# rrahn/libspm

Hardware: AMD Instinct MI355X
Metric: Gbases/s scanned, Myers k<=3 |P|=100 (higher is better)
Workload: dtype u32

## Files before the change

### libspm_amd/csrc/filter_verify.hip

```cpp
#include "filter_launch.hpp"
#include "filter_verify.hpp"

namespace
{
template <int NWN>
void launch_verify_nw(const verify_params &V, dim3 grid, hipStream_t s)
{
    uint32_t threads = 256;
    const size_t per_thread = (size_t)(V.sigma + 1) * NWN * 4 + 2 * 16;
    while (threads > 64 && per_thread * threads > 128 * 1024)
        threads >>= 1;
    const size_t lds = per_thread * threads + (size_t)(threads / 64) * kHitStage * sizeof(spm_hit);
    launch(verify_kernel<NWN>, grid, threads, lds, s, V);
}

template <int G>
void launch_verify_wave_g(verify_params V, const uint32_t *peq_bot, uint32_t max_m, dim3 grid, hipStream_t s)
{
    grid.x *= 4;
    const uint32_t n_slots = 2 * V.max_k + 1 + V.max_span;
    V.wave_text = ((max_m + V.max_k + n_slots + 16 + 15) & ~15u) + 16;
    const size_t per_group = ((n_slots * 2 + 15) & ~15u) + V.wave_text;
    launch(verify_wave_kernel<G, 1>, grid, 64, (64 / G) * per_group, s, V, peq_bot);
}
}

void launch_band_runs(const verify_params &V, band_rec *bands, band_rec *heads, unsigned long long *head_count, uint32_t n_cu,
                      hipStream_t s)
{
    hipLaunchKernelGGL(band_runs_kernel, dim3(n_cu * 8), dim3(256), 0, s, V, bands, heads, head_count);
}

void launch_band_select(const verify_params &V, band_rec *out, unsigned long long *out_count, uint32_t n_cu, hipStream_t s)
{
    hipLaunchKernelGGL(band_select_kernel, dim3(n_cu * 2), dim3(256), 0, s, V, out, out_count);
}

void launch_band_release(const verify_params &V, const band_rec *bands, uint32_t n_cu, hipStream_t s)
{
    hipLaunchKernelGGL(band_release_kernel, dim3(n_cu * 8), dim3(256), 0, s, V, bands, (uint32_t)kCntBandSlots);
}

void launch_verify_wave(uint32_t n_blocks, const verify_params &V, const uint32_t *peq_bot, uint32_t max_m, uint32_t n_cu,
                        hipStream_t s)
{
    const dim3 grid(n_cu * 16);
    if (n_blocks <= 8)
        launch_verify_wave_g<8>(V, peq_bot, max_m, grid, s);
    else if (n_blocks <= 16)
        launch_verify_wave_g<16>(V, peq_bot, max_m, grid, s);
    else if (n_blocks <= 32)
        launch_verify_wave_g<32>(V, peq_bot, max_m, grid, s);
    else
        launch_verify_wave_g<64>(V, peq_bot, max_m, grid, s);
}

void launch_verify(uint32_t nwn, const verify_params &V, uint64_t band_expect, uint32_t n_cu, hipStream_t s)
{
    const dim3 grid((uint32_t)std::min<uint64_t>((uint64_t)n_cu * 4, std::max<uint64_t>(n_cu / 2, (band_expect + 255) / 256)));
    switch (nwn) {
    case 1: launch_verify_nw<1>(V, grid, s); break;
    case 2: launch_verify_nw<2>(V, grid, s); break;
    case 3: launch_verify_nw<3>(V, grid, s); break;
    case 4: launch_verify_nw<4>(V, grid, s); break;
    case 5: launch_verify_nw<5>(V, grid, s); break;
    case 6: launch_verify_nw<6>(V, grid, s); break;
    case 7: launch_verify_nw<7>(V, grid, s); break;
    case 8: launch_verify_nw<8>(V, grid, s); break;
    case 16: launch_verify_nw<16>(V, grid, s); break;
    case 32: launch_verify_nw<32>(V, grid, s); break;
    default: launch_verify_nw<64>(V, grid, s); break;
    }
}

void warm_verify_kernels()
{
    hipFuncAttributes a;
    (void)hipFuncGetAttributes(&a, (const void *)band_release_kernel);
}
```

### libspm_amd/csrc/filter_verify.hpp

```cpp
#pragma once

#include "brute.hpp"
#include "filter_params.hpp"
#include "pack.hpp"
#include "wave.hpp"

namespace spm_hip
{

__device__ __forceinline__ bool seen_insert(const verify_params &P, uint32_t pat, int64_t e)
{
    return seen_insert_raw(P.seen, P.seen_mask, P.overflow, pat, e);
}

__global__ __launch_bounds__(256) void band_select_kernel(const verify_params P, band_rec *out, unsigned long long *out_count)
{
    unsigned long long n = P.counters[kCntBandSlots];
    if (n > P.band_cap)
        n = P.band_cap;
    const uint32_t lane = threadIdx.x & 63;
    const uint64_t stride = (uint64_t)gridDim.x * blockDim.x;
    const uint64_t rounds = (n + stride - 1) / stride;
    for (uint64_t r = 0; r < rounds; ++r) {
        const uint64_t i = r * stride + (uint64_t)blockIdx.x * blockDim.x + threadIdx.x;
        bool keep = false;
        band_rec c;
        c.val = kBandInvalid;
        if (i < n) {
            c = P.bands[i];
            if (c.val != kBandInvalid) {
                const uint32_t cnt = (uint32_t)band_value(P.band_tab[c.slot].y, true);
                band_release(P.band_tab, c.slot);
                keep = cnt >= (P.surplus ? (uint32_t)P.surplus[c.val >> 11] : 1u);
            }
        }
        const uint64_t m = __ballot(keep);
        if (m != 0) {
            unsigned long long base = 0;
            const int leader = __ffsll((unsigned long long)m) - 1;
            if ((int)lane == leader)
                base = atomicAdd(out_count, (unsigned long long)__popcll(m));
            base = __shfl(base, leader);
            if (keep)
                out[base + __popcll(m & ((1ull << lane) - 1))] = c;
        }
    }
}

constexpr uint32_t kRunAnalysed = 0x400u;
constexpr uint32_t kRunFollower = 0x200u;
constexpr uint32_t kRunLenShift = 5, kRunLenMask = 0x3u, kRunHiMask = 0x1Fu;
constexpr uint32_t kRunTouchLeft = 0x80u, kRunTouchRight = 0x100u;
constexpr uint32_t kRunMax = 4;

__device__ __forceinline__ uint32_t band_lookup(const verify_params &P, unsigned long long bkey)
{
    uint32_t s2 = (uint32_t)mix64(bkey) & P.table_mask;
    for (uint32_t tries = 0; tries < 8192; ++tries) {
        const unsigned long long o = P.band_tab[s2].x;
        if (o == bkey)
            return s2;
        if (o == kBandEmpty)
            return 0xFFFFFFFFu;
        s2 = (s2 + 1) & P.table_mask;
    }
    return 0xFFFFFFFFu;
}

__global__ __launch_bounds__(256) void band_runs_kernel(const verify_params P, band_rec *bands, band_rec *heads,
                                                        unsigned long long *head_count)
{
    __shared__ uint32_t wave_tot01[4], wave_tot23[4];
    __shared__ unsigned long long chunk_base;
    unsigned long long n = P.counters[P.band_counter];
    if (n > P.band_cap)
        n = P.band_cap;
    constexpr uint32_t PER = 8;
    const uint32_t tid = threadIdx.x, lane = tid & 63, wave = tid >> 6;
    for (uint64_t c0 = (uint64_t)blockIdx.x * (256 * PER); c0 < n; c0 += (uint64_t)gridDim.x * (256 * PER)) {
        band_rec mine[PER];
        uint32_t head_mask = 0, cnt = 0;
#pragma unroll
        for (uint32_t j = 0; j < PER; ++j) {
            const uint64_t i = c0 + (uint64_t)j * 256 + tid;
            mine[j].val = kBandInvalid;
            if (i >= n)
                continue;
            band_rec c = bands[i];
            if (c.val == kBandInvalid)
                continue;
            const unsigned long long base = ((unsigned long long)(c.val >> 11) << 43) | ((unsigned long long)c.seg << P.band_bits);
            uint32_t code = kRunAnalysed;
            const bool pred = c.band > 0 && band_lookup(P, base | (unsigned long long)(c.band - 1)) != 0xFFFFFFFFu;
            if (c.band % kRunMax != 0 && pred) {
                code |= kRunFollower;
            } else {
                uint32_t followers = 0, last = c.slot;
                bool cut = true;
                for (uint32_t r = 1; r < kRunMax && (c.band + r) % kRunMax != 0; ++r) {
                    const uint32_t s2 = band_lookup(P, base | (unsigned long long)(c.band + r));
                    if (s2 == 0xFFFFFFFFu) {
                        cut = false;
                        break;
                    }
                    followers = r;
                    last = s2;
                }
                const bool succ = cut && band_lookup(P, base | (unsigned long long)(c.band + followers + 1)) != 0xFFFFFFFFu;
                const unsigned long long v = band_value(P.band_tab[last].y, false);
                const uint32_t hi = v ? (uint32_t)(63 - __clzll((long long)v)) : 0u;
                code |= (followers << kRunLenShift) | (hi & kRunHiMask) | (pred ? kRunTouchLeft : 0u) | (succ ? kRunTouchRight : 0u);
                head_mask |= 1u << j;
                ++cnt;
            }
            c.val = (c.val & ~0x7FFu) | code;
            mine[j] = c;
        }
        uint32_t c01 = 0, c23 = 0;
#pragma unroll
        for (uint32_t j = 0; j < PER; ++j)
            if (head_mask & (1u << j)) {
                const uint32_t cls = (mine[j].val >> kRunLenShift) & kRunLenMask;
                const uint32_t one = 1u << (16 * (cls & 1u));
                c01 += cls < 2 ? one : 0u;
                c23 += cls < 2 ? 0u : one;
            }
        uint32_t i01 = c01, i23 = c23;
#pragma unroll
        for (int o = 1; o < 64; o <<= 1) {
            const uint32_t u01 = (uint32_t)__shfl_up((int)i01, o), u23 = (uint32_t)__shfl_up((int)i23, o);
            if (lane >= (uint32_t)o) {
                i01 += u01;
                i23 += u23;
            }
        }
        if (lane == 63) {
            wave_tot01[wave] = i01;
            wave_tot23[wave] = i23;
        }
        __syncthreads();
        uint32_t off01 = 0, off23 = 0, tot01 = 0, tot23 = 0;
        for (uint32_t w = 0; w < 4; ++w) {
            off01 += w < wave ? wave_tot01[w] : 0u;
            off23 += w < wave ? wave_tot23[w] : 0u;
            tot01 += wave_tot01[w];
            tot23 += wave_tot23[w];
        }
        const uint32_t tot[4] = {tot01 & 0xFFFFu, tot01 >> 16, tot23 & 0xFFFFu, tot23 >> 16};
        const uint32_t total = tot[0] + tot[1] + tot[2] + tot[3];
        if (tid == 0)
            chunk_base = total ? atomicAdd(head_count, (unsigned long long)total) : 0ull;
        __syncthreads();
        const uint32_t mine_before[4] = {(off01 & 0xFFFFu) + ((i01 - c01) & 0xFFFFu), (off01 >> 16) + ((i01 - c01) >> 16),
                                         (off23 & 0xFFFFu) + ((i23 - c23) & 0xFFFFu), (off23 >> 16) + ((i23 - c23) >> 16)};
        uint64_t pos[4];
        pos[0] = chunk_base + mine_before[0];
        pos[1] = chunk_base + tot[0] + mine_before[1];
        pos[2] = chunk_base + tot[0] + tot[1] + mine_before[2];
        pos[3] = chunk_base + tot[0] + tot[1] + tot[2] + mine_before[3];
#pragma unroll
        for (uint32_t j = 0; j < PER; ++j)
            if (head_mask & (1u << j)) {
                const uint32_t cls = (mine[j].val >> kRunLenShift) & kRunLenMask;
                const uint64_t at = cls == 0 ? pos[0] : cls == 1 ? pos[1] : cls == 2 ? pos[2] : pos[3];
                heads[at] = mine[j];
                pos[0] += cls == 0 ? 1u : 0u;
                pos[1] += cls == 1 ? 1u : 0u;
                pos[2] += cls == 2 ? 1u : 0u;
                pos[3] += cls == 3 ? 1u : 0u;
            }
        __syncthreads();
    }
}

__global__ __launch_bounds__(256) void band_release_kernel(const verify_params P, const band_rec *bands, uint32_t counter)
{
    unsigned long long n = P.counters[counter];
    if (n > P.band_cap)
        n = P.band_cap;
    const uint64_t stride = (uint64_t)gridDim.x * blockDim.x;
    for (uint64_t i = (uint64_t)blockIdx.x * blockDim.x + threadIdx.x; i < n; i += stride) {
        const band_rec c = bands[i];
        if (c.val != kBandInvalid)
            band_release(P.band_tab, c.slot);
    }
}

struct band_geom
{
    uint32_t pat;
    int64_t m, k;
    int64_t e_lo, e_hi;
    int64_t ws;
    int64_t dd_lo, dd_hi;
};

__device__ __forceinline__ bool decode_band(const verify_params &P, const band_rec &c, bool consume, band_geom &g)
{
    if (c.val == kBandInvalid)
        return false;
    g.pat = c.val >> 11;
    unsigned long long v = 1;
    if (!P.preselected) {
        v = band_value(P.band_tab[c.slot].y, P.overlap != 0);
        if (consume)
            band_release(P.band_tab, c.slot);
        if (c.val & kRunFollower)
            return false;
        if (P.overlap ? (uint32_t)v < (P.surplus ? (uint32_t)P.surplus[g.pat] : 1u) : v == 0)
            return false;
    }
    g.m = P.m[g.pat];
    g.k = P.k[g.pat];
    int64_t own_b = (int64_t)P.scan_begin, own_e = (int64_t)P.scan_end, hay_b = (int64_t)P.ctx_begin;
    if (P.seg_offsets) {
        const int64_t sb = (int64_t)P.seg_offsets[c.seg], se = (int64_t)P.seg_offsets[c.seg + 1];
        own_b = P.seg_owned ? sb + (int64_t)P.seg_owned[c.seg] : sb;
        own_e = se;
        hay_b = sb;
    }
    const int64_t band_base = hay_b - (int64_t)P.max_m + (int64_t)c.band * (int64_t)P.Bw;
    int64_t d = band_base;
    int64_t span = (int64_t)P.Bw - 1 + (P.overlap ? g.k + 1 : 0);
    if (!P.overlap) {
        const int lo = __ffsll((long long)v) - 1;
        int hi = 63 - __clzll((long long)v);
        if (c.val & kRunAnalysed)
            hi = (int)(((c.val >> kRunLenShift) & kRunLenMask) * P.Bw + (c.val & kRunHiMask));
        d += lo;
        span = hi - lo;
    }
    g.e_lo = d + g.m - g.k;
    g.e_hi = d + g.m + g.k + span;
    g.dd_lo = INT64_MAX;
    g.dd_hi = INT64_MIN;
    if (!P.overlap && (c.val & kRunAnalysed) && !P.seg_offsets) {
        const int64_t next_base = band_base + (int64_t)(((c.val >> kRunLenShift) & kRunLenMask) + 1) * (int64_t)P.Bw;
        g.dd_lo = (c.val & kRunTouchLeft) ? band_base + g.m + g.k : INT64_MIN;
        g.dd_hi = (c.val & kRunTouchRight) ? next_base + g.m - g.k - 1 : INT64_MAX;
    }
    if (g.e_lo < own_b + 1)
        g.e_lo = own_b + 1;
    if (g.e_hi > own_e)
        g.e_hi = own_e;
    if (g.e_lo > g.e_hi)
        return false;
    g.ws = g.e_lo - (g.m + g.k);
    if (g.ws < hay_b)
        g.ws = hay_b;
    return true;
}

template <int NWN>
__global__ __launch_bounds__(256) void verify_kernel(const verify_params P)
{
    extern __shared__ uint32_t vlds[];
    const uint32_t tid = threadIdx.x;
    const uint32_t nthr = blockDim.x;
    const uint32_t rows = P.sigma + 1;
    uint16_t *hitbuf = reinterpret_cast<uint16_t *>(vlds + (size_t)rows * NWN * nthr);
    spm_hit *stage = reinterpret_cast<spm_hit *>(hitbuf + (size_t)16 * nthr) + (size_t)(tid >> 6) * kHitStage;
    uint32_t n_staged = 0;
    const uint32_t lane = tid & 63;
    auto flush = [&]() {
        if (n_staged == 0)
            return;
        unsigned long long base = 0;
        if (lane == 0)
            base = atomicAdd(P.hit_counter, (unsigned long long)n_staged);
        base = uniform_u64(base);
        for (uint32_t i = lane; i < n_staged; i += 64)
            if (base + i < P.hit_cap)
                P.hits[base + i] = stage[i];
        n_staged = 0;
        queue_sync();
    };
    unsigned long long n_cand = P.counters[P.band_counter];
    if (n_cand > P.band_cap)
        n_cand = P.band_cap;
    const uint64_t stride = (uint64_t)gridDim.x * nthr;
    uint32_t n_valid = 0;
    const uint64_t rounds = (n_cand + stride - 1) / stride;
    for (uint64_t rd = 0; rd < rounds; ++rd) {
        const uint64_t ci = rd * stride + (uint64_t)blockIdx.x * nthr + tid;
        band_geom g;
        g.pat = 0;
        g.m = 1;
        g.k = 0;
        g.e_lo = 0;
        g.e_hi = -1;
        g.ws = 0;
        const bool active = ci < n_cand && decode_band(P, P.bands[ci], P.runs == 0, g);
        if (active)
            ++n_valid;
        const uint32_t pat = g.pat;
        const int64_t m = g.m, k = g.k, e_lo = g.e_lo, e_hi = active ? g.e_hi : g.ws, ws = g.ws;
        const uint32_t *src = P.peq32 + (((size_t)(pat >> 6) * rows) * P.nw_table + (P.nw_table - NWN)) * 64 + (pat & 63);
        if (active)
            for (uint32_t r = 0; r < rows; ++r)
#pragma unroll
                for (int w = 0; w < NWN; ++w)
                    vlds[((size_t)r * NWN + w) * nthr + tid] = src[((size_t)r * P.nw_table + w) * 64];
        myers_lane<NWN, false> L;
        {
            const int32_t off = NWN * 32 - (int32_t)m;
#pragma unroll
            for (int w = 0; w < NWN; ++w) {
                const int32_t lo = off - w * 32;
                L.VP[w] = lo <= 0 ? 0xFFFFFFFFu : (lo >= 32 ? 0u : (0xFFFFFFFFu << lo));
                L.VN[w] = 0;
            }
            L.score = (int32_t)m;
        }
        const int64_t blk0 = ws & ~15ll;
        uint4 nxt = make_uint4(0, 0, 0, 0);
        if (active)
            nxt = load_text16(P.text, (uint64_t)blk0, P.text_alloc);
        const uint32_t n_cols = (uint32_t)(e_hi - ws);
        const uint32_t rel_lo = (uint32_t)(e_lo - 1 - ws);
        const uint32_t sigma = P.sigma;
        uint32_t rel0 = (uint32_t)(blk0 - ws);
        const uint32_t my_blocks = active ? (uint32_t)((e_hi - blk0 + 15) >> 4) : 0u;
        uint32_t max_blocks = my_blocks;
        for (int o = 32; o > 0; o >>= 1)
            max_blocks = max(max_blocks, (uint32_t)__shfl_xor((int)max_blocks, o));
        max_blocks = (uint32_t)__builtin_amdgcn_readfirstlane(max_blocks);
        for (uint32_t bi = 0; bi < max_blocks; ++bi, rel0 += 16) {
            const int64_t blk = blk0 + 16 * (int64_t)bi;
            uint32_t hitmask = 0;
            if (bi < my_blocks) {
                const uint4 cur = nxt;
                if (bi + 1 < my_blocks)
                    nxt = load_text16(P.text, (uint64_t)(blk + 16), P.text_alloc);
                const uint32_t words[4] = {cur.x, cur.y, cur.z, cur.w};
#pragma unroll
                for (int i = 0; i < 16; ++i) {
                    const uint32_t rel = rel0 + (uint32_t)i;
                    if (rel >= n_cols)
                        continue;
                    uint32_t sym = (words[i >> 2] >> (8 * (i & 3))) & 0xFF;
                    sym = sym < sigma ? sym : sigma;
                    L.step_strided(vlds + ((size_t)sym * NWN) * nthr + tid, nthr);
                    if (L.score <= (int32_t)k && rel >= rel_lo) {
                        hitbuf[(size_t)i * nthr + tid] = (uint16_t)(L.score + 1);
                        hitmask |= 1u << i;
                    }
                }
            }
            if (__ballot(hitmask != 0) == 0)
                continue;
            uint32_t fresh = 0, keep = 0;
            for (uint32_t mm = hitmask; mm != 0; mm &= mm - 1) {
                const uint32_t i = (uint32_t)__ffs(mm) - 1u;
                const int64_t e = blk + (int64_t)i + 1;
                if ((e > g.dd_lo && e < g.dd_hi) || seen_insert(P, pat, e)) {
                    ++fresh;
                    keep |= 1u << i;
                }
            }
            uint32_t incl = fresh;
#pragma unroll
            for (int o = 1; o < 64; o <<= 1) {
                const uint32_t up = (uint32_t)__shfl_up((int)incl, o);
                if (lane >= (uint32_t)o)
                    incl += up;
            }
            const uint32_t total = (uint32_t)__builtin_amdgcn_readfirstlane(__shfl((int)incl, 63));
            if (total == 0)
                continue;
            if (n_staged + total > kHitStage)
                flush();
            unsigned long long direct = 0;
            const bool staged = total <= kHitStage;
            if (!staged) {
                if (lane == 0)
                    direct = atomicAdd(P.hit_counter, (unsigned long long)total);
                direct = uniform_u64(direct);
            }
            uint32_t at = n_staged + incl - fresh;
            for (uint32_t mm = keep; mm != 0; mm &= mm - 1) {
                const uint32_t i = (uint32_t)__ffs(mm) - 1u;
                const int64_t e = blk + (int64_t)i + 1;
                spm_hit h;
                h.pos = (P.report_begin ? (uint64_t)(e - m) : (uint64_t)e) + P.pos_offset;
                h.pattern = pat;
                h.score = (int32_t)hitbuf[(size_t)i * nthr + tid] - 1;
                if (staged)
                    stage[at] = h;
                else if (direct + at < P.hit_cap)
                    P.hits[direct + at] = h;
                ++at;
            }
            if (staged)
                n_staged += total;
            queue_sync();
        }
    }
    flush();
    wave_count_add(P.hit_counter + kCntBandsVerified, n_valid);
}


template <int G, int NB>
__global__ __launch_bounds__(256) void verify_wave_kernel(const verify_params P, const uint32_t *__restrict__ peq_bot)
{
    extern __shared__ uint16_t whit[];
    constexpr uint32_t GPW = 64 / G;
    const uint32_t lane = threadIdx.x & 63, gl = lane & (G - 1), gw = lane / G;
    const uint32_t wave = threadIdx.x >> 6, waves = blockDim.x >> 6;
    const uint32_t n_slots = 2 * P.max_k + 1 + P.max_span;
    const uint32_t group_bytes = ((n_slots * 2 + 15) & ~15u) + P.wave_text;
    uint8_t *gbase = reinterpret_cast<uint8_t *>(whit) + (size_t)(wave * GPW + gw) * group_bytes;
    uint16_t *hb = reinterpret_cast<uint16_t *>(gbase);
    uint8_t *tw = gbase + ((n_slots * 2 + 15) & ~15u);
    for (uint32_t r = gl; r < n_slots; r += G)
        hb[r] = 0;
    unsigned long long n_cand = P.counters[P.band_counter];
    if (n_cand > P.band_cap)
        n_cand = P.band_cap;
    const uint64_t stride = (uint64_t)gridDim.x * waves * GPW;
    const uint32_t rows = P.sigma + 1;
    uint32_t n_valid = 0;
    for (uint64_t base = ((uint64_t)blockIdx.x * waves + wave) * GPW; base < n_cand; base += stride) {
        const uint64_t ci = base + gw;
        bool active = ci < n_cand;
        uint32_t pat = 0;
        int64_t m = 1, k = 0, e_lo = 0, e_hi = -1, ws = 0;
        band_rec c;
        c.val = kBandInvalid;
        c.slot = 0;
        if (active)
            c = P.bands[ci];
        {
            band_geom g;
            g.pat = 0;
            g.m = 1;
            g.k = 0;
            g.e_lo = 0;
            g.e_hi = -1;
            g.ws = 0;
            active = active && decode_band(P, c, false, g);
            pat = g.pat;
            m = g.m;
            k = g.k;
            e_lo = g.e_lo;
            e_hi = g.e_hi;
            ws = g.ws;
        }
        __builtin_amdgcn_wave_barrier();
        if (gl == 0 && c.val != kBandInvalid && !P.preselected)
            band_release(P.band_tab, c.slot);
        if (active && gl == 0)
            ++n_valid;
        const uint32_t nbk = (uint32_t)((m + 31) >> 5);
        const uint32_t nb = (nbk + NB - 1) / NB;
        const uint32_t n_cols = active ? (uint32_t)(e_hi - ws) : 0u;
        const bool mine = active && gl < nb;
        const bool lane_last = gl + 1 == nb;
        const uint32_t j_last = (nbk - 1) % NB;
        uint32_t out_bit[NB];
#pragma unroll
        for (int j = 0; j < NB; ++j)
            out_bit[j] = (gl * NB + (uint32_t)j + 1 == nbk) ? (uint32_t)((m - 1) & 31) : 31u;
        const uint32_t skew = (uint32_t)(ws & 15);
        uint32_t beyond4 = 0;
        if (active) {
            const uint32_t n_bytes = (skew + n_cols + 15) & ~15u;
            for (uint32_t off = gl * 16; off < n_bytes; off += G * 16) {
                const uint4 v = load_text16(P.text, ((uint64_t)ws & ~15ull) + off, P.text_alloc);
                *reinterpret_cast<uint4 *>(tw + off) = v;
                beyond4 |= (v.x | v.y | v.z | v.w) & 0xFCFCFCFCu;
            }
        }
        const bool plain4 = P.sigma == 4 && __ballot(beyond4 != 0) == 0;
        uint32_t e0[NB], e1[NB], e2[NB], e3[NB], e4[NB];
#pragma unroll
        for (int j = 0; j < NB; ++j) {
            e0[j] = e1[j] = e2[j] = e3[j] = e4[j] = 0;
            const uint32_t gb = gl * NB + (uint32_t)j;
            if (mine && gb < nbk) {
                const uint32_t *src = peq_bot + (((size_t)(pat >> 6) * rows) * P.nw_table + gb) * 64 + (pat & 63);
                const size_t rs = (size_t)P.nw_table * 64;
                e0[j] = src[0];
                e1[j] = src[rs];
                e2[j] = P.sigma > 2 ? src[2 * rs] : 0u;
                e3[j] = P.sigma > 3 ? src[3 * rs] : 0u;
                e4[j] = P.sigma > 4 ? src[4 * rs] : 0u;
            }
        }
        queue_sync();
        uint32_t Pv[NB], Mv[NB], ho = 0;
#pragma unroll
        for (int j = 0; j < NB; ++j) {
            Pv[j] = 0xFFFFFFFFu;
            Mv[j] = 0;
        }
        int32_t score = (int32_t)m;
        bool any_hit = false;
        const uint32_t first_slot_col = (uint32_t)(e_lo - ws) - 1;
        const uint32_t t_end = n_cols + nb - 1;
        uint32_t t_wave = active ? t_end : 0u;
        uint32_t t_lo = active ? nb - 1 : 0u, t_hi = active ? n_cols : 0xFFFFFFFFu;
        uint32_t t_hit = active ? first_slot_col + nb - 1 : 0xFFFFFFFFu;
        for (int o = 32; o >= (int)G; o >>= 1) {
            t_wave = max(t_wave, (uint32_t)__shfl_xor((int)t_wave, o));
            t_lo = max(t_lo, (uint32_t)__shfl_xor((int)t_lo, o));
            t_hi = min(t_hi, (uint32_t)__shfl_xor((int)t_hi, o));
            t_hit = min(t_hit, (uint32_t)__shfl_xor((int)t_hit, o));
        }
        t_wave = (uint32_t)__builtin_amdgcn_readfirstlane(t_wave);
        t_lo = (uint32_t)__builtin_amdgcn_readfirstlane(t_lo);
        t_hi = (uint32_t)__builtin_amdgcn_readfirstlane(t_hi);
        t_hit = (uint32_t)__builtin_amdgcn_readfirstlane(t_hit);
        t_hi = t_hi > t_wave ? t_wave : t_hi;
        t_lo = t_lo > t_hi ? t_hi : t_lo;
        t_hit = t_hit < t_lo ? t_lo : (t_hit > t_hi ? t_hi : t_hit);
        uint32_t sym_next = mine ? tw[skew] : 0u;
        const uint8_t *my_text = mine ? tw + skew - gl : tw;
        const int32_t k_hit = (lane_last && mine) ? (int32_t)k : -1;
        const uint32_t n_rel = n_cols - first_slot_col;
        auto step = [&](uint32_t t, auto checked, auto dna4, auto hits) {
            const uint32_t ho_up = (uint32_t)__builtin_amdgcn_update_dpp(0, (int)ho, 0x138, 0xF, 0xF, false);
            const uint32_t col = t - gl;
            const uint32_t sym = sym_next;
            if constexpr (decltype(checked)::value) {
                uint32_t nc = col + 1;
                nc = nc < n_cols ? nc : 0u;
                sym_next = tw[skew + nc];
            } else {
                sym_next = my_text[t + 1];
            }
            if (!decltype(checked)::value || (mine && col < n_cols)) {
                uint32_t hin = gl == 0 ? 0u : ho_up;
                uint32_t s0 = 0, s1 = 0;
                if constexpr (decltype(dna4)::value) {
                    s0 = (uint32_t)((int32_t)(sym << 31) >> 31);
                    s1 = (uint32_t)((int32_t)(sym << 30) >> 31);
                }
                int32_t d_last = 0;
#pragma unroll
                for (int j = 0; j < NB; ++j) {
                    uint32_t Eq;
                    if constexpr (decltype(dna4)::value) {
                        const uint32_t lo2 = (e1[j] & s0) | (e0[j] & ~s0), hi2 = (e3[j] & s0) | (e2[j] & ~s0);
                        Eq = (hi2 & s1) | (lo2 & ~s1);
                    } else {
                        const uint32_t lo2 = (sym & 1u) ? e1[j] : e0[j], hi2 = (sym & 1u) ? e3[j] : e2[j];
                        Eq = (sym & 2u) ? hi2 : lo2;
                        Eq = sym < 4 ? Eq : (sym == 4 ? e4[j] : 0u);
                        Eq = sym < P.sigma ? Eq : 0u;
                    }
                    const uint32_t hp = hin & 1u, hn = hin >> 1;
                    const uint32_t Xv = Eq | Mv[j];
                    Eq |= hn;
                    const uint32_t Xh = (((Eq & Pv[j]) + Pv[j]) ^ Pv[j]) | Eq;
                    uint32_t Ph = Mv[j] | ~(Xh | Pv[j]);
                    uint32_t Mh = Pv[j] & Xh;
                    const uint32_t op = (Ph >> out_bit[j]) & 1u, on = (Mh >> out_bit[j]) & 1u;
                    hin = op | (on << 1);
                    Ph = (Ph << 1) | hp;
                    Mh = (Mh << 1) | hn;
                    Pv[j] = Mh | ~(Xv | Ph);
                    Mv[j] = Ph & Xv;
                    if (NB == 1 || (uint32_t)j == j_last)
                        d_last = (int32_t)op - (int32_t)on;
                }
                ho = hin;
                score += d_last;
                if constexpr (decltype(hits)::value) {
                    const uint32_t rel = col - first_slot_col;
                    if (score <= k_hit && rel < n_rel) {
                        hb[rel] = (uint16_t)(score + 1);
                        any_hit = true;
                    }
                }
            }
        };
        uint32_t t = 0;
        for (; t < t_lo; ++t)
            step(t, std::true_type{}, std::false_type{}, std::true_type{});
        if (plain4) {
            for (; t < t_hit; ++t)
                step(t, std::false_type{}, std::true_type{}, std::false_type{});
            for (; t < t_hi; ++t)
                step(t, std::false_type{}, std::true_type{}, std::true_type{});
        } else {
            for (; t < t_hi; ++t)
                step(t, std::false_type{}, std::false_type{}, std::true_type{});
        }
        for (; t < t_wave; ++t)
            step(t, std::true_type{}, std::false_type{}, std::true_type{});
        queue_sync();
        if (__ballot(any_hit) != 0) {
            const uint32_t nr = active ? (uint32_t)(e_hi - e_lo) + 1 : 0u;
            uint32_t fresh = 0;
            for (uint32_t r = gl; r < nr; r += G) {
                const uint32_t sc1 = hb[r];
                if (sc1) {
                    if (seen_insert(P, pat, e_lo + (int64_t)r))
                        ++fresh;
                    else
                        hb[r] = 0;
                }
            }
            unsigned long long idx = wave_reserve_hits(P.hit_counter, fresh);
            for (uint32_t r = gl; r < nr; r += G) {
                const uint32_t sc1 = hb[r];
                hb[r] = 0;
                if (sc1) {
                    if (idx < P.hit_cap) {
                        const int64_t e = e_lo + (int64_t)r;
                        spm_hit h;
                        h.pos = (P.report_begin ? (uint64_t)(e - m) : (uint64_t)e) + P.pos_offset;
                        h.pattern = pat;
                        h.score = (int32_t)sc1 - 1;
                        P.hits[idx] = h;
                    }
                    ++idx;
                }
            }
        }
        queue_sync();
    }
    wave_count_add(P.hit_counter + kCntBandsVerified, n_valid);
}

}
```

Before: 6533.

## Replace register Eq select with LDS symbol table lookup in wave verify kernel

The wave verify kernel now stores each lane's per-symbol pattern-match words in an LDS table indexed by symbol, replacing the register-held e0..e4 arrays and the branchless select logic. Text bytes are clamped so out-of-range symbols map to a zero row, which removes the separate DNA4/plain path. The Eq word for the next column is prefetched one step ahead, the horizontal carries pass as separate DPP values with sign-extended bit extraction, and the unchecked loop is manually unrolled by four. The NB multi-block-per-lane template is dropped. This adds LDS traffic per step and extra table storage per launch, in exchange for fewer ALU ops in the inner recurrence.

```diff
diff --git a/libspm_amd/csrc/filter_verify.hip b/libspm_amd/csrc/filter_verify.hip
--- a/libspm_amd/csrc/filter_verify.hip
+++ b/libspm_amd/csrc/filter_verify.hip
@@ -21,7 +21,7 @@
     const uint32_t n_slots = 2 * V.max_k + 1 + V.max_span;
     V.wave_text = ((max_m + V.max_k + n_slots + 16 + 15) & ~15u) + 16;
     const size_t per_group = ((n_slots * 2 + 15) & ~15u) + V.wave_text;
-    launch(verify_wave_kernel<G, 1>, grid, 64, (64 / G) * per_group, s, V, peq_bot);
+    launch(verify_wave_kernel<G>, grid, 64, (64 / G) * per_group + kWaveTableBytes, s, V, peq_bot);
 }
 }
 
diff --git a/libspm_amd/csrc/filter_verify.hpp b/libspm_amd/csrc/filter_verify.hpp
--- a/libspm_amd/csrc/filter_verify.hpp
+++ b/libspm_amd/csrc/filter_verify.hpp
@@ -401,7 +401,18 @@
 }
 
 
-template <int G, int NB>
+constexpr uint32_t kWaveSymRows = 8;
+constexpr uint32_t kWaveTableBytes = kWaveSymRows * 64 * 4;
+
+__device__ __forceinline__ uint32_t clamp_syms(uint32_t w)
+{
+    const uint32_t hi = w & 0xF8F8F8F8u;
+    const uint32_t any = ((hi | (hi >> 1) | (hi >> 2) | (hi >> 3) | (hi >> 4)) >> 3) & 0x01010101u;
+    const uint32_t full = any * 0xFFu;
+    return (w & ~full) | (0x07070707u & full);
+}
+
+template <int G>
 __global__ __launch_bounds__(256) void verify_wave_kernel(const verify_params P, const uint32_t *__restrict__ peq_bot)
 {
     extern __shared__ uint16_t whit[];
@@ -413,8 +424,12 @@
     uint8_t *gbase = reinterpret_cast<uint8_t *>(whit) + (size_t)(wave * GPW + gw) * group_bytes;
     uint16_t *hb = reinterpret_cast<uint16_t *>(gbase);
     uint8_t *tw = gbase + ((n_slots * 2 + 15) & ~15u);
+    uint32_t *tabl = reinterpret_cast<uint32_t *>(reinterpret_cast<uint8_t *>(whit) + (size_t)waves * GPW * group_bytes +
+                                                  (size_t)wave * kWaveTableBytes) + lane;
     for (uint32_t r = gl; r < n_slots; r += G)
         hb[r] = 0;
+    for (uint32_t off = gl * 16; off < P.wave_text; off += G * 16)
+        *reinterpret_cast<uint4 *>(tw + off) = make_uint4(0, 0, 0, 0);
     unsigned long long n_cand = P.counters[P.band_counter];
     if (n_cand > P.band_cap)
         n_cand = P.band_cap;
@@ -452,49 +467,31 @@
             band_release(P.band_tab, c.slot);
         if (active && gl == 0)
             ++n_valid;
-        const uint32_t nbk = (uint32_t)((m + 31) >> 5);
-        const uint32_t nb = (nbk + NB - 1) / NB;
+        const uint32_t nb = (uint32_t)((m + 31) >> 5);
         const uint32_t n_cols = active ? (uint32_t)(e_hi - ws) : 0u;
         const bool mine = active && gl < nb;
         const bool lane_last = gl + 1 == nb;
-        const uint32_t j_last = (nbk - 1) % NB;
-        uint32_t out_bit[NB];
-#pragma unroll
-        for (int j = 0; j < NB; ++j)
-            out_bit[j] = (gl * NB + (uint32_t)j + 1 == nbk) ? (uint32_t)((m - 1) & 31) : 31u;
+        const uint32_t out_bit = lane_last ? (uint32_t)((m - 1) & 31) : 31u;
         const uint32_t skew = (uint32_t)(ws & 15);
-        uint32_t beyond4 = 0;
         if (active) {
             const uint32_t n_bytes = (skew + n_cols + 15) & ~15u;
             for (uint32_t off = gl * 16; off < n_bytes; off += G * 16) {
-                const uint4 v = load_text16(P.text, ((uint64_t)ws & ~15ull) + off, P.text_alloc);
+                uint4 v = load_text16(P.text, ((uint64_t)ws & ~15ull) + off, P.text_alloc);
+                if ((v.x | v.y | v.z | v.w) & 0xF8F8F8F8u)
+                    v = make_uint4(clamp_syms(v.x), clamp_syms(v.y), clamp_syms(v.z), clamp_syms(v.w));
                 *reinterpret_cast<uint4 *>(tw + off) = v;
-                beyond4 |= (v.x | v.y | v.z | v.w) & 0xFCFCFCFCu;
-            }
-        }
-        const bool plain4 = P.sigma == 4 && __ballot(beyond4 != 0) == 0;
-        uint32_t e0[NB], e1[NB], e2[NB], e3[NB], e4[NB];
-#pragma unroll
-        for (int j = 0; j < NB; ++j) {
-            e0[j] = e1[j] = e2[j] = e3[j] = e4[j] = 0;
-            const uint32_t gb = gl * NB + (uint32_t)j;
-            if (mine && gb < nbk) {
-                const uint32_t *src = peq_bot + (((size_t)(pat >> 6) * rows) * P.nw_table + gb) * 64 + (pat & 63);
-                const size_t rs = (size_t)P.nw_table * 64;
-                e0[j] = src[0];
-                e1[j] = src[rs];
-                e2[j] = P.sigma > 2 ? src[2 * rs] : 0u;
-                e3[j] = P.sigma > 3 ? src[3 * rs] : 0u;
-                e4[j] = P.sigma > 4 ? src[4 * rs] : 0u;
-            }
+            }
+        }
+        {
+            const uint32_t *src = peq_bot + (((size_t)(pat >> 6) * rows) * P.nw_table + gl) * 64 + (pat & 63);
+            const size_t rs = (size_t)P.nw_table * 64;
+#pragma unroll
+            for (uint32_t r = 0; r < kWaveSymRows; ++r)
+                tabl[r * 64] = (mine && r < P.sigma) ? src[r * rs] : 0u;
         }
         queue_sync();
-        uint32_t Pv[NB], Mv[NB], ho = 0;
-#pragma unroll
-        for (int j = 0; j < NB; ++j) {
-            Pv[j] = 0xFFFFFFFFu;
-            Mv[j] = 0;
-        }
+        uint32_t Pv = 0xFFFFFFFFu, Mv = 0;
+        uint32_t op_c = 0, on_c = 0;
         int32_t score = (int32_t)m;
         bool any_hit = false;
         const uint32_t first_slot_col = (uint32_t)(e_lo - ws) - 1;
@@ -515,58 +512,38 @@
         t_hi = t_hi > t_wave ? t_wave : t_hi;
         t_lo = t_lo > t_hi ? t_hi : t_lo;
         t_hit = t_hit < t_lo ? t_lo : (t_hit > t_hi ? t_hi : t_hit);
-        uint32_t sym_next = mine ? tw[skew] : 0u;
         const uint8_t *my_text = mine ? tw + skew - gl : tw;
         const int32_t k_hit = (lane_last && mine) ? (int32_t)k : -1;
         const uint32_t n_rel = n_cols - first_slot_col;
-        auto step = [&](uint32_t t, auto checked, auto dna4, auto hits) {
-            const uint32_t ho_up = (uint32_t)__builtin_amdgcn_update_dpp(0, (int)ho, 0x138, 0xF, 0xF, false);
+        const uint32_t carry_in = gl == 0 ? 0u : 1u;
+        uint32_t eq_cur = tabl[(uint32_t)tw[skew] * 64];
+        uint32_t sym_nx = tw[skew + ((1u - gl) < n_cols ? 1u - gl : 0u)];
+        auto step = [&](uint32_t t, auto checked, auto hits) {
             const uint32_t col = t - gl;
-            const uint32_t sym = sym_next;
+            const uint32_t eq_nx = tabl[sym_nx * 64];
             if constexpr (decltype(checked)::value) {
-                uint32_t nc = col + 1;
+                uint32_t nc = col + 2;
                 nc = nc < n_cols ? nc : 0u;
-                sym_next = tw[skew + nc];
+                sym_nx = tw[skew + nc];
             } else {
-                sym_next = my_text[t + 1];
-            }
+                sym_nx = my_text[t + 2];
+            }
+            const uint32_t hp = (uint32_t)__builtin_amdgcn_update_dpp(0, (int)op_c, 0x138, 0xF, 0xF, true) & carry_in;
+            const uint32_t hn = (uint32_t)__builtin_amdgcn_update_dpp(0, (int)on_c, 0x138, 0xF, 0xF, true) & carry_in;
             if (!decltype(checked)::value || (mine && col < n_cols)) {
-                uint32_t hin = gl == 0 ? 0u : ho_up;
-                uint32_t s0 = 0, s1 = 0;
-                if constexpr (decltype(dna4)::value) {
-                    s0 = (uint32_t)((int32_t)(sym << 31) >> 31);
-                    s1 = (uint32_t)((int32_t)(sym << 30) >> 31);
-                }
-                int32_t d_last = 0;
-#pragma unroll
-                for (int j = 0; j < NB; ++j) {
-                    uint32_t Eq;
-                    if constexpr (decltype(dna4)::value) {
-                        const uint32_t lo2 = (e1[j] & s0) | (e0[j] & ~s0), hi2 = (e3[j] & s0) | (e2[j] & ~s0);
-                        Eq = (hi2 & s1) | (lo2 & ~s1);
-                    } else {
-                        const uint32_t lo2 = (sym & 1u) ? e1[j] : e0[j], hi2 = (sym & 1u) ? e3[j] : e2[j];
-                        Eq = (sym & 2u) ? hi2 : lo2;
-                        Eq = sym < 4 ? Eq : (sym == 4 ? e4[j] : 0u);
-                        Eq = sym < P.sigma ? Eq : 0u;
-                    }
-                    const uint32_t hp = hin & 1u, hn = hin >> 1;
-                    const uint32_t Xv = Eq | Mv[j];
-                    Eq |= hn;
-                    const uint32_t Xh = (((Eq & Pv[j]) + Pv[j]) ^ Pv[j]) | Eq;
-                    uint32_t Ph = Mv[j] | ~(Xh | Pv[j]);
-                    uint32_t Mh = Pv[j] & Xh;
-                    const uint32_t op = (Ph >> out_bit[j]) & 1u, on = (Mh >> out_bit[j]) & 1u;
-                    hin = op | (on << 1);
-                    Ph = (Ph << 1) | hp;
-                    Mh = (Mh << 1) | hn;
-                    Pv[j] = Mh | ~(Xv | Ph);
-                    Mv[j] = Ph & Xv;
-                    if (NB == 1 || (uint32_t)j == j_last)
-                        d_last = (int32_t)op - (int32_t)on;
-                }
-                ho = hin;
-                score += d_last;
+                uint32_t Eq = eq_cur;
+                const uint32_t Xv = Eq | Mv;
+                Eq |= hn;
+                const uint32_t Xh = (((Eq & Pv) + Pv) ^ Pv) | Eq;
+                uint32_t Ph = Mv | ~(Xh | Pv);
+                uint32_t Mh = Pv & Xh;
+                op_c = __builtin_amdgcn_ubfe(Ph, out_bit, 1);
+                on_c = (uint32_t)__builtin_amdgcn_sbfe((int)Mh, out_bit, 1);
+                score += (int32_t)op_c + (int32_t)on_c;
+                Ph = (Ph << 1) | hp;
+                Mh = (Mh << 1) | hn;
+                Pv = Mh | ~(Xv | Ph);
+                Mv = Ph & Xv;
                 if constexpr (decltype(hits)::value) {
                     const uint32_t rel = col - first_slot_col;
                     if (score <= k_hit && rel < n_rel) {
@@ -575,21 +552,29 @@
                     }
                 }
             }
+            eq_cur = eq_nx;
+        };
+        auto run_unchecked = [&](uint32_t &t, uint32_t to, auto hits) {
+#pragma clang loop unroll(disable)
+            for (; t + 4 <= to; t += 4) {
+                step(t, std::false_type{}, hits);
+                step(t + 1, std::false_type{}, hits);
+                step(t + 2, std::false_type{}, hits);
+                step(t + 3, std::false_type{}, hits);
+            }
+#pragma clang loop unroll(disable)
+            for (; t < to; ++t)
+                step(t, std::false_type{}, hits);
         };
         uint32_t t = 0;
+#pragma clang loop unroll(disable)
         for (; t < t_lo; ++t)
-            step(t, std::true_type{}, std::false_type{}, std::true_type{});
-        if (plain4) {
-            for (; t < t_hit; ++t)
-                step(t, std::false_type{}, std::true_type{}, std::false_type{});
-            for (; t < t_hi; ++t)
-                step(t, std::false_type{}, std::true_type{}, std::true_type{});
-        } else {
-            for (; t < t_hi; ++t)
-                step(t, std::false_type{}, std::false_type{}, std::true_type{});
-        }
+            step(t, std::true_type{}, std::true_type{});
+        run_unchecked(t, t_hit, std::false_type{});
+        run_unchecked(t, t_hi, std::true_type{});
+#pragma clang loop unroll(disable)
         for (; t < t_wave; ++t)
-            step(t, std::true_type{}, std::false_type{}, std::true_type{});
+            step(t, std::true_type{}, std::true_type{});
         queue_sync();
         if (__ballot(any_hit) != 0) {
             const uint32_t nr = active ? (uint32_t)(e_hi - e_lo) + 1 : 0u;
```

Result: no change. 6532 (median of 2 runs) (-0.0%).
